# wdecoster/inquiSTR

Measured on AMD Instinct MI355X. Metric: loci/sec genotyped (inquiSTR call hot path, device-resident batch = L0), higher is better.
Workload: dtype u32/i64; 1 GPU; unphased100k: 100000 loci/GPU x 30 reads x ~200 CIGAR ops, --unphased, device-resident SoA (L0); loci_per_gpu=100000, pairs_per_gpu=3000000, cigar_ops_per_gpu=600007253, minlen=5, support=3, total_loci=100000

## Files before the change

inquistr_amd/csrc/capi.hip:

```cpp
#include <hip/hip_runtime.h>

#include <algorithm>
#include <cmath>
#include <cstdio>
#include <cstring>
#include <new>
#include <string>
#include <thread>
#include <vector>

#include "../../include/inquistr_hip.h"
#include "cigar_walk.h"
#include "ctx.h"
#include "evidence.h"
#include "front_kernels.h"
#include "kernels.h"
#include "locus_motifs.h"
#include "read_calls.h"
#include "read_motifs.h"
#include "read_seqs.h"

using namespace inq;

namespace inq {
// ... 66 lines not shown
    b.cap = got;
    return INQ_OK;
}

int upload(inq_ctx *c, hipStream_t s, std::initializer_list<Upload> ups) {
    for (const Upload &u : ups) {
        const int rc = ensure(c, *u.d, u.bytes);
        if (rc != INQ_OK) return rc;
        if (u.bytes) HIP_TRY(c, hipMemcpyAsync(u.d->p, u.h, u.bytes, hipMemcpyHostToDevice, s));
    }
    return INQ_OK;
}

int status_to_code(uint32_t st) {
    if (st & ST_HINT) return INQ_ERR_ARG;
    if (st & ST_LOCUS) return INQ_ERR_LOCUS;
    if (st & ST_INDEX) return INQ_ERR_INDEX;
    if (st & ST_CIGAR_OP) return INQ_ERR_CIGAR_OP;
    if (st & ST_RANGE) return INQ_ERR_RANGE;
    if (st & ST_PHASE) return INQ_ERR_PHASE;
    if (st & ST_AUX) return INQ_ERR_AUX;
    if (st & ST_INTERNAL) return INQ_ERR_HIP;
    return INQ_OK;
}

int status_readback(inq_ctx *c, DevStatus *dst, hipStream_t s) {
    HIP_TRY(c, hipMemcpyAsync(dst, c->d_status, sizeof(DevStatus), hipMemcpyDeviceToHost, s));
    HIP_TRY(c, hipMemsetAsync(&c->d_status->err, 0, sizeof(unsigned int), s));
    HIP_TRY(c, hipMemsetAsync(&c->d_status->ties, 0, sizeof(unsigned long long), s));
    return INQ_OK;
}

DevBatch device_batch(const void *cigar, const void *reads, const void *pair_read, const void *off, const void *lstart, const void *lend,
                      uint64_t n_reads, uint64_t n_cigar_words, uint64_t n_pairs, uint64_t n_loci, uint32_t minlen, uint32_t support,
                      uint32_t unphased, void *p1, void *p2, void *pair_call, void *pair_bits) {
    DevBatch d;
    d.b = {n_reads, n_cigar_words, n_pairs, n_loci, (const uint32_t *)cigar, (const inq_read_t *)reads, (const uint32_t *)pair_read,
           (const uint64_t *)off, (const uint32_t *)lstart, (const uint32_t *)lend, minlen, support, unphased, 0u};
    d.r = {(double *)p1, (double *)p2, (int64_t *)pair_call, (uint8_t *)pair_bits, 0};
    return d;
}

static int timing_begin(inq_ctx *c, hipStream_t s, EvTriple **ev) {
    *ev = nullptr;
    if (!c->timing) return INQ_OK;
    if (c->ev_used == c->ev_pool.size()) {
        EvTriple t;
        HIP_TRY(c, hipEventCreate(&t.e0));
        HIP_TRY(c, hipEventCreate(&t.e1));
        HIP_TRY(c, hipEventCreate(&t.e2));
        c->ev_pool.push_back(t);
    }
    *ev = &c->ev_pool[c->ev_used++];
    HIP_TRY(c, hipEventRecord((*ev)->e0, s));
    return INQ_OK;
}

}

extern "C" {

int inq_abi_version(void) { return INQ_ABI_VERSION; }

const char *inq_strerror(int code) {
    switch (code) {
    case INQ_OK: return "ok";
    case INQ_ERR_ARG: return "invalid argument (null pointer, inconsistent sizes or non-monotone offsets)";
    case INQ_ERR_SUPPORT_ZERO: return "support must be >= 1";
    case INQ_ERR_PHASE: return "a read passing the phased filter has HP outside {0,1,2}";
    case INQ_ERR_CIGAR_OP: return "CIGAR op code above 8";
    case INQ_ERR_LOCUS: return "locus start < 10 or end < start";
    case INQ_ERR_RANGE: return "read position plus reference span does not fit 31 bits";
    case INQ_ERR_INDEX: return "pair or CIGAR index outside the batch buffers";
    case INQ_ERR_HIP: return "HIP runtime error";
    case INQ_ERR_NOMEM: return "out of device memory";
    case INQ_ERR_INFLATE: return "a BGZF block does not inflate to its recorded size (corrupt or truncated BAM)";
    case INQ_ERR_BAM: return "corrupt BAM record chain, or records not coordinate-sorted";
    case INQ_ERR_AUX: return "HP aux of a fetched read is neither C nor i, or the SA aux of a kept read with a soft clip cannot be parsed (the reference panics)";
    case INQ_ERR_NO_DEVICE: return "no gfx950 (MI355X) device available; this library has no CPU fallback";
    default: return "unknown error";
    }
}

static void apply_default_options(inq_ctx *c);
static bool default_option(const char *key, int64_t *value);

int inq_ctx_create_early(int device_id, inq_ctx_t **out, volatile int *stage_ready) {
    if (!out) return INQ_ERR_ARG;
    *out = nullptr;
    if (stage_ready) *stage_ready = 0;
    int n = 0;
    HostClock clock("[inq ctx]");
    if (hipGetDeviceCount(&n) != hipSuccess || n <= 0) return INQ_ERR_NO_DEVICE;
    clock.lap("hipGetDeviceCount (runtime init)");
    if (device_id < 0 || device_id >= n) return INQ_ERR_ARG;
    hipDeviceProp_t prop;
    if (hipGetDeviceProperties(&prop, device_id) != hipSuccess) return INQ_ERR_HIP;
    if (std::strncmp(prop.gcnArchName, "gfx950", 6) != 0) return INQ_ERR_NO_DEVICE;
    inq_ctx *c = new (std::nothrow) inq_ctx();
    if (!c) return INQ_ERR_NOMEM;
    c->device = device_id;
    c->n_cus = (uint32_t)std::max(prop.multiProcessorCount, 1);
    c->grid_tail = std::min<uint32_t>(c->grid_tail, c->n_cus);
    c->backend = std::string("hip:") + prop.gcnArchName + ":" + prop.name;
    bool published = false;
    auto fail = [&](int code) {
// ... 124 lines not shown
    if (!x.kept_off != !x.kept || ((uintptr_t)x.kept & 15u) || ((uintptr_t)x.kept_off & 7u)) return INQ_ERR_ARG;
    if (x.kept && b->n_pairs && (!r->pair_call || !r->pair_bits)) return INQ_ERR_ARG;
    if (x.names.recs && (!x.kept || !x.names.off || !x.name_off || ((uintptr_t)x.names.recs & 7u))) return INQ_ERR_ARG;
    if (x.seqs.recs && (!x.kept || !x.kept_pair || !x.seqs.off || !x.seq_qbeg || !x.seq_len || ((uintptr_t)x.seqs.recs & 7u))) return INQ_ERR_ARG;
    if (((uintptr_t)b->cigar & 15u) || ((uintptr_t)b->reads & 15u)) return INQ_ERR_ARG;
    HIP_TRY(c, hipSetDevice(c->device));
    hipStream_t s = hip_stream ? (hipStream_t)hip_stream : c->stream;
    const uint64_t blocks = (b->n_loci + 3) / 4;
    const uint32_t per_xcd = (uint32_t)((blocks + 7) / 8);
    const uint32_t grid_small = per_xcd * 8u;
    const uint32_t shard_cap = (grid_small / kListShards + 1u) * 4u;
    if ((rc = ensure(c, c->worklist, (size_t)shard_cap * kListShards * kListKinds * 4)) != INQ_OK) return rc;
    if ((rc = ensure(c, c->sval, (size_t)b->n_pairs * 8)) != INQ_OK) return rc;
    if ((rc = ensure(c, c->smeta, (size_t)b->n_pairs)) != INQ_OK) return rc;
    const uint32_t hint = c->call_hint ? c->call_hint : c->max_reads_hint;
    const bool deep_possible = b->n_pairs > kGridSelectMin && !(hint && hint <= kGridSelectMin);
    if (deep_possible && (rc = ensure(c, c->deep, deep_select_scratch_bytes(b->n_pairs))) != INQ_OK) return rc;
    const uint64_t ev_list_cap = x.evidence && b->n_pairs > kEvidenceWaveMax && !(hint && hint <= kEvidenceWaveMax) ? evidence_list_cap(b->n_pairs) : 0;
    if (x.evidence && (rc = ensure(c, c->evwork, evidence_scratch_bytes(ev_list_cap))) != INQ_OK) return rc;
    if (x.kept && b->n_pairs && (rc = ensure(c, c->rctiles, read_call_scratch_bytes(b->n_pairs))) != INQ_OK) return rc;

    KArgs a;
    a.cigar4 = (const uint4 *)b->cigar;
    a.reads = (const uint4 *)b->reads;
    a.pair_read = b->pair_read;
    a.locus_pair_off = b->locus_pair_off;
    a.locus_start = b->locus_start;
    a.locus_end = b->locus_end;
    a.n_reads = b->n_reads;
    a.n_cigar4 = b->n_cigar_words / 4;
    a.n_pairs = b->n_pairs;
    a.n_loci = b->n_loci;
    a.minlen = b->minlen;
    a.support = b->support;
    a.phase1 = r->phase1;
    a.phase2 = r->phase2;
    a.pair_call = r->pair_call;
    a.pair_bits = r->pair_bits;
    a.status = c->d_status;
    a.worklist = (uint32_t *)c->worklist.p;
    a.sval = (int64_t *)c->sval.p;
    a.smeta = (uint8_t *)c->smeta.p;
    a.blocks_per_xcd = per_xcd;
    a.shard_cap = shard_cap;
    c->call_hint = 0;
    a.max_reads_hint = hint;
    a.locus_flags = x.flags;

    const bool nt = c->nt_loads < 0 ? (b->n_pairs <= b->n_reads) : (c->nt_loads != 0);
    EvTriple *ev;
    if ((rc = timing_begin(c, s, &ev)) != INQ_OK) return rc;
    if (x.flags) HIP_TRY(c, hipMemsetAsync(x.flags, 0, (size_t)b->n_loci, s));
    if (x.evidence) HIP_TRY(c, hipMemsetAsync(c->evwork.p, 0, sizeof(EvidenceWork), s));
    launch_locus_call(a, b->unphased != 0, nt, grid_small, c->grid_medium, c->grid_tail, s, ev ? ev->e1 : nullptr, deep_possible ? c->deep.p : nullptr);
    HIP_TRY(c, hipGetLastError());
    const PairView view{b->locus_pair_off, r->pair_bits, r->pair_call, b->pair_read, (const uint32_t *)b->reads, b->n_reads, b->n_pairs, b->n_loci};
    if (x.evidence) {
        EvidenceWork *const work = (EvidenceWork *)c->evwork.p;
        launch_evidence(EvidenceArgs{view, x.evidence, work, (EvidenceSlice *)(work + 1), ev_list_cap}, b->unphased != 0, c->n_cus * 4u, s);
        HIP_TRY(c, hipGetLastError());
    }
    if (x.kept && !b->n_pairs) HIP_TRY(c, hipMemsetAsync(x.kept_off, 0, (size_t)(b->n_loci + 1) * 8, s));
    if (x.kept && b->n_pairs) {
        uint64_t *const tile_base = (uint64_t *)c->rctiles.p;
        launch_read_calls(ReadCallArgs{view, x.kept_off, x.kept, (uint32_t *)(tile_base + read_call_tiles(b->n_pairs) + 1), tile_base, x.kept_pair},
                          b->unphased != 0, s);
        HIP_TRY(c, hipGetLastError());
    }
    const uint64_t *const n_kept = x.kept_off ? x.kept_off + b->n_loci : nullptr;
    auto place_runs = [&](const auto &runs, auto &&records) {
        if (!runs.recs) return hipSuccess;
        if (!b->n_pairs) return hipMemsetAsync(runs.off, 0, 8, s);
        records();
        launch_scan_run_bytes(runs.recs, n_kept, runs.off, b->n_pairs, runs.off + b->n_pairs + 1, s);
        return hipGetLastError();
    };
    const auto origins = [&] { launch_read_origins(ReadOriginArgs{x.kept, n_kept, view.read_words, b->n_reads, x.name_off, x.names.recs, b->n_pairs}, c->grid_side, s); };
    const auto slices = [&] { launch_read_seq_records(ReadSeqArgs{x.kept_pair, n_kept, x.seq_qbeg, x.seq_len, x.seqs.recs, b->n_pairs}, c->grid_side, s); };
    HIP_TRY(c, place_runs(x.names, origins));
    HIP_TRY(c, place_runs(x.seqs, slices));
    const KeptSlices kept{x.kept_pair, n_kept, x.kept_off, b->n_loci, x.seq_bytes, x.seq_n_bytes, x.seq_off, x.seq_len, b->n_pairs, b->n_pairs};
    if (x.locus_found && !b->n_pairs) HIP_TRY(c, hipMemsetAsync(x.locus_found, 0, (size_t)b->n_loci * sizeof(inq_locus_motif_t), s));
    if (x.locus_found && b->n_pairs) {
        launch_locus_motifs(LocusMotifArgs{kept, x.motif_given, x.locus_found, x.motif_use}, c->grid_side, s);
        HIP_TRY(c, hipGetLastError());
    }
    if (x.motifs && b->n_pairs) {
        launch_read_motifs(ReadMotifArgs{kept, x.motif_word, x.motifs}, c->grid_side, s);
        HIP_TRY(c, hipGetLastError());
    }
    if (ev) HIP_TRY(c, hipEventRecord(ev->e2, s));
    return INQ_OK;
}

int inq_call_batch_device(inq_ctx_t *c, const inq_batch_t *b, inq_result_t *r, void *hip_stream) {
    return inq_call_batch_device_flags(c, b, r, nullptr, hip_stream);
}

int inq_call_batch_device_flags(inq_ctx_t *c, const inq_batch_t *b, inq_result_t *r, uint8_t *d_locus_flags, void *hip_stream) {
    return inq_call_batch_device_evidence(c, b, r, d_locus_flags, nullptr, hip_stream);
}

int inq_call_batch_device_evidence(inq_ctx_t *c, const inq_batch_t *b, inq_result_t *r, uint8_t *d_locus_flags, inq_locus_evidence_t *d_evidence,
                                   void *hip_stream) {
    return inq_call_batch_device_reads(c, b, r, d_locus_flags, d_evidence, nullptr, nullptr, hip_stream);
}

int inq_call_batch_device_reads(inq_ctx_t *c, const inq_batch_t *b, inq_result_t *r, uint8_t *d_locus_flags, inq_locus_evidence_t *d_evidence,
                                uint64_t *d_kept_off, inq_read_call_t *d_kept, void *hip_stream) {
    return guarded([&] { return enqueue_batch(c, b, r, hip_stream, LocusExtras{d_locus_flags, d_evidence, d_kept_off, d_kept}); });
}

int inq_ctx_status(inq_ctx_t *c, uint64_t *n_tie_loci) {
    if (!c) return INQ_ERR_ARG;
    HIP_TRY(c, hipSetDevice(c->device));
    HIP_TRY(c, hipDeviceSynchronize());
    const int rc = status_readback(c, c->h_status, c->stream);
    if (rc != INQ_OK) return rc;
    HIP_TRY(c, hipStreamSynchronize(c->stream));
    if (n_tie_loci) *n_tie_loci = c->h_status->ties;
    return status_to_code(c->h_status->err);
}

static int call_batch_impl(inq_ctx_t *c, const inq_batch_t *b, inq_result_t *r, const HostExtras &h) {
    if (!c) return INQ_ERR_ARG;
    extras_reset(c);
    int rc = check_scalars(b, r);
    if (rc != INQ_OK) return rc;
    uint64_t max_reads = 0;
    if (b->n_loci) {
        const uint64_t *const off = b->locus_pair_off;
        if (off[0] != 0 || off[b->n_loci] != b->n_pairs || !offsets_ok(off, b->n_loci, b->n_pairs)) return INQ_ERR_ARG;
        for (uint64_t j = 0; j < b->n_loci; ++j) {
            if (!locus_ok(b->locus_start[j], b->locus_end[j])) return INQ_ERR_LOCUS;
            max_reads = std::max<uint64_t>(max_reads, b->locus_pair_off[j + 1] - b->locus_pair_off[j]);
        }
    }
    r->n_tie_loci = 0;
    if (b->n_loci == 0) {
        extras_finish(c, 0, 0, h, 0);
        return INQ_OK;
    }
    HIP_TRY(c, hipSetDevice(c->device));
    hipStream_t s = c->stream;
// ... 158 lines not shown
        if (firth_when) {
            launch_assoc_firth(a, s);
            HIP_TRY(c, hipGetLastError());
        }
        if (ev) {
            HIP_TRY(c, hipEventRecord(ev->e1, s));
            HIP_TRY(c, hipEventRecord(ev->e2, s));
        }
        HIP_TRY(c, hipMemcpyAsync(rows + r0, c->arows.p, a.n_rows * sizeof(inq_assoc_row_t), hipMemcpyDeviceToHost, s));
        if (firth_when) HIP_TRY(c, hipMemcpyAsync(firth + r0, c->afirth.p, a.n_rows * sizeof(inq_assoc_firth_row_t), hipMemcpyDeviceToHost, s));
    }
    HIP_TRY(c, hipStreamSynchronize(s));
    return INQ_OK;
}

int inq_assoc_rows(inq_ctx_t *c, const float *values, uint64_t n_rows, uint32_t n_samples, const double *y, const double *cov, uint32_t k,
                   int outcome, int str_mode, double missing_cutoff, inq_assoc_row_t *rows) {
    return guarded([&] { return assoc_rows_impl(c, values, n_rows, n_samples, y, cov, k, outcome, str_mode, missing_cutoff, rows); });
}

int inq_assoc_rows_firth(inq_ctx_t *c, const float *values, uint64_t n_rows, uint32_t n_samples, const double *y, const double *cov,
                         uint32_t k, int str_mode, double missing_cutoff, int when, inq_assoc_row_t *rows, inq_assoc_firth_row_t *firth) {
    if (when != INQ_ASSOC_FIRTH_FALLBACK && when != INQ_ASSOC_FIRTH_ALWAYS) return INQ_ERR_ARG;
    return guarded([&] { return assoc_rows_impl(c, values, n_rows, n_samples, y, cov, k, INQ_ASSOC_BINARY, str_mode, missing_cutoff, rows, when, firth); });
}

int inq_ctx_timing_enable(inq_ctx_t *c, int on) {
    if (!c) return INQ_ERR_ARG;
    c->timing = on != 0;
    return INQ_OK;
}

int inq_ctx_timing_reset(inq_ctx_t *c) {
    if (!c) return INQ_ERR_ARG;
    HIP_TRY(c, hipSetDevice(c->device));
    HIP_TRY(c, hipDeviceSynchronize());
    c->ev_used = 0;
    return INQ_OK;
}

int inq_ctx_timing_read(inq_ctx_t *c, int which, double *total_ms, uint64_t *launches) {
    if (!c || which < 0 || which > 2) return INQ_ERR_ARG;
    HIP_TRY(c, hipSetDevice(c->device));
    if (which == 2) {
        HIP_TRY(c, hipDeviceSynchronize());
        const double ms = span_last_inflate_ms(c->span);
        if (total_ms) *total_ms = ms < 0 ? 0.0 : ms;
        if (launches) *launches = ms < 0 ? 0u : 1u;
        return INQ_OK;
    }
    double tot = 0.0;
    for (size_t i = 0; i < c->ev_used; ++i) {
        EvTriple &e = c->ev_pool[i];
        HIP_TRY(c, hipEventSynchronize(e.e2));
        float ms = 0.f;
        HIP_TRY(c, hipEventElapsedTime(&ms, e.e0, which == 0 ? e.e2 : e.e1));
        tot += (double)ms;
    }
    if (total_ms) *total_ms = tot;
    if (launches) *launches = (uint64_t)c->ev_used;
    return INQ_OK;
}

static std::mutex g_defaults_mu;
static std::vector<std::pair<std::string, int64_t>> g_defaults;

int inq_default_option(const char *key, int64_t value) {
    if (!key) return INQ_ERR_ARG;
    try {
        inq_ctx probe;
        probe.n_cus = 256;
        const int rc = inq_ctx_set_option(&probe, key, value);
        if (rc != INQ_OK) return rc;
        std::lock_guard<std::mutex> g(g_defaults_mu);
        for (auto &kv : g_defaults)
            if (kv.first == key) {
                kv.second = value;
                return INQ_OK;
            }
        g_defaults.emplace_back(key, value);
        return INQ_OK;
    } catch (...) {
        return INQ_ERR_NOMEM;
    }
}

static bool default_option(const char *key, int64_t *value) {
    std::lock_guard<std::mutex> g(g_defaults_mu);
    for (auto &kv : g_defaults)
        if (kv.first == key) {
            if (value) *value = kv.second;
            return true;
        }
    return false;
}
int inq_default_option_get(const char *key, int64_t *value) {
    if (!key) return INQ_ERR_ARG;
    try {
        return default_option(key, value) ? INQ_OK : INQ_ERR_ARG;
    } catch (...) {
        return INQ_ERR_NOMEM;
    }
}

static void apply_default_options(inq_ctx *c) {
    std::vector<std::pair<std::string, int64_t>> d;
    {
        std::lock_guard<std::mutex> g(g_defaults_mu);
        d = g_defaults;
// ... 123 lines not shown
```

inquistr_amd/csrc/cigar_walk.h:

```cpp
#pragma once
#include <type_traits>

#include "wave_primitives.h"

namespace inq {

typedef unsigned int u32x4 __attribute__((ext_vector_type(4)));

constexpr uint32_t ST_INDEX = 1u, ST_CIGAR_OP = 2u, ST_RANGE = 4u, ST_PHASE = 8u, ST_LOCUS = 16u, ST_HINT = 32u, ST_AUX = 64u,
                   ST_INTERNAL = 128u;

constexpr uint32_t PM_CLIP = 1u, PM_FETCHED = 2u, PM_KEPT = 4u;
constexpr int PM_GRP_SHIFT = 4;
constexpr uint32_t PM_CHOSEN = 64u;

constexpr uint32_t RB_UNMAPPED = 1u, RB_REVERSE = 2u, RB_HAS_HP = 4u, RB_IS_2D = 8u, RB_SA_PANIC = 16u;

constexpr int kQueueCap = 128;

struct Window {
    uint32_t se;
    uint32_t ee;
    uint32_t se1;
    uint32_t width;
// ... 53 lines not shown
    if (lane < cnt) {
        uint32_t ri = b.pair_read[first + (uint64_t)lane];
        if ((uint64_t)ri < b.n_reads) {
            uint4 r = b.reads[ri];
            uint64_t n4 = ((uint64_t)r.y + 3u) >> 2;
            if (r.y < 0x10000000u && (uint64_t)r.x + n4 <= b.n_cigar4) {
                m.off4 = r.x;
                m.nc = r.y | ((r.w & (RB_IS_2D << 8)) ? 0x80000000u : 0u);
                m.pos = r.z;
                m.misc = r.w;
                valid = true;
            } else {
                status |= ST_INDEX;
            }
        } else {
            status |= ST_INDEX;
        }
    }
    return m;
}

__device__ __forceinline__ uint32_t meta_stage_a(const BatchView &b, uint64_t first, int cnt, int lane) {
    return lane < cnt ? b.pair_read[first + (uint64_t)lane] : 0xffffffffu;
}
__device__ __forceinline__ uint4 meta_stage_b(const BatchView &b, uint32_t ri) {
    return (uint64_t)ri < b.n_reads ? b.reads[ri] : make_uint4(0u, 0xffffffffu, 0u, 0u);
}
__device__ __forceinline__ PairMeta meta_stage_c(const BatchView &b, const uint4 r, int cnt, int lane, uint32_t &status,
                                                  bool &valid) {
    PairMeta m{0u, 0u, 0u, 0u};
    valid = false;
    if (lane < cnt) {
        const uint64_t n4 = ((uint64_t)r.y + 3u) >> 2;
        if (r.y < 0x10000000u && (uint64_t)r.x + n4 <= b.n_cigar4) {
            m.off4 = r.x;
            m.nc = r.y | ((r.w & (RB_IS_2D << 8)) ? 0x80000000u : 0u);
            m.pos = r.z;
            m.misc = r.w;
            valid = true;
        } else {
            status |= ST_INDEX;
        }
    }
    return m;
}

constexpr uint32_t kConsume = 0x18Du;

__device__ __forceinline__ uint32_t ref_advance(uint32_t op, uint32_t len) {
    return len & (uint32_t)__builtin_amdgcn_sbfe((int)kConsume, op, 1u);
}
constexpr uint32_t kConsume32 = kConsume | (kConsume << 16);
__device__ __forceinline__ uint32_t ref_advance_raw(uint32_t w) {
    return (w >> 4) & (uint32_t)__builtin_amdgcn_sbfe((int)kConsume32, w, 1u);
}
constexpr uint32_t kBadOp32 = 0xFE00FE00u;
__device__ __forceinline__ uint32_t bad_ops(const u32x4 w) {
    return (kBadOp32 >> (w.x & 31u)) | (kBadOp32 >> (w.y & 31u)) | (kBadOp32 >> (w.z & 31u)) | (kBadOp32 >> (w.w & 31u));
}
__device__ __forceinline__ void advance4(const u32x4 w, uint32_t &e1, uint32_t &e2, uint32_t &e3, uint32_t &tot) {
    e1 = ref_advance_raw(w.x), e2 = e1 + ref_advance_raw(w.y);
    e3 = e2 + ref_advance_raw(w.z), tot = e3 + ref_advance_raw(w.w);
}

__device__ __forceinline__ void drain_queue(WaveLds &L, uint32_t &qcount, const Window &W, int lane) {
    __builtin_amdgcn_wave_barrier();
    for (uint32_t base = 0; base < qcount; base += 64u) {
        const uint32_t e = base + (uint32_t)lane;
        if (e < qcount) {
            const u32x4 w = L.q[e].w;
            const uint2 info = L.q[e].info;
            const uint32_t rel = info.x;
            const uint32_t slot = info.y & 63u;
            const uint32_t cand_mask = (info.y & 64u) ? 0x06u : 0x16u;
            const uint32_t op0 = w.x & 15u, op1 = w.y & 15u, op2 = w.z & 15u, op3 = w.w & 15u;
            const uint32_t l0 = w.x >> 4, l1 = w.y >> 4, l2 = w.z >> 4, l3 = w.w >> 4;
            const uint32_t e1 = ref_advance(op0, l0), e2 = e1 + ref_advance(op1, l1), e3 = e2 + ref_advance(op2, l2);
            int32_t s = 0;
            uint32_t clip = 0;
#define INQ_OP(op, len, ee_)                                                                              \
    {                                                                                                     \
        const bool hit = ((cand_mask >> (op)) & 1u) && (len) > W.minlen && (rel + (ee_)) < W.width;        \
        const int32_t v = ((op) == 2u) ? -(int32_t)(len) : (int32_t)(len);                                \
        s += hit ? v : 0;                                                                                 \
        clip |= (hit && (op) == 4u) ? 1u : 0u;                                                            \
    }
            INQ_OP(op0, l0, 0u)
            INQ_OP(op1, l1, e1)
            INQ_OP(op2, l2, e2)
            INQ_OP(op3, l3, e3)
#undef INQ_OP
            if (s != 0) atomicAdd(&L.acc[slot], (unsigned long long)(long long)s);
            if (clip) atomicOr(&L.flags[slot], 1u);
        }
    }
    qcount = 0;
    __builtin_amdgcn_wave_barrier();
}

__device__ __forceinline__ bool push_window_lanes(WaveLds &L, uint32_t &qcount, bool inw, const u32x4 w, uint32_t x,
                                                  uint32_t tot, uint32_t info, uint32_t info_mask) {
    const uint64_t mask = ballot64(inw);
    if (mask) {
        QueueEntry *const tail = &L.q[qcount];
        if (inw) {
            const uint32_t idx = __builtin_amdgcn_mbcnt_hi((uint32_t)(mask >> 32), __builtin_amdgcn_mbcnt_lo((uint32_t)mask, 0u));
            tail[idx].w = w;
// ... 367 lines not shown
```

inquistr_amd/csrc/ctx.h:

```cpp
#pragma once
#include <hip/hip_runtime.h>

#include <array>
#include <chrono>
#include <cstdio>
#include <cstdlib>
#include <initializer_list>
#include <mutex>
#include <new>
#include <string>
#include <utility>
#include <vector>

#include "../../include/inquistr_hip.h"
#include "kernels.h"

namespace inq {

struct DevBuf {
    void *p = nullptr;
    size_t cap = 0;
};

struct EvTriple {
    hipEvent_t e0, e1, e2;
};

struct KeptRuns {
    DevBuf recs, off, bytes;
    uint64_t n_recs = 0, n_bytes = 0;
    auto bufs() { return std::array{&recs, &off, &bytes}; }
};

struct SpanState;

}

struct inq_ctx {
    int device = -1;
    hipStream_t stream = nullptr;
    std::string backend, last_err;
    inq::DevStatus *d_status = nullptr;
    inq::DevStatus *h_status = nullptr;
    inq::DevBuf worklist, sval, smeta, deep;
    inq::DevBuf cigar, reads, pair_read, off, lstart, lend, p1, p2, pcall, pbits, lflags;
    inq::DevBuf levidence, evwork;
    inq::DevBuf rctiles, rcoff, rckept;
    uint64_t read_calls_total = 0;
    inq::KeptRuns rnames, rseqs;
    inq::DevBuf rkeptpair;
    inq::DevBuf rmotifs, rmotifword;
    uint64_t read_motifs_total = 0;
    inq::DevBuf rlocusmotif, rmotifuse;
    inq::DevBuf ovalues, olen, oflags, okeep, otrans;
    inq::DevBuf avalues, ay, acov, atcoef, arows;
    inq::DevBuf aminmu, afirth;
    auto bufs() {
        std::vector<inq::DevBuf *> all{&worklist, &sval, &smeta, &deep, &cigar, &reads, &pair_read, &off, &lstart, &lend, &p1, &p2, &pcall, &pbits,
                                       &lflags, &levidence, &evwork, &rctiles, &rcoff, &rckept, &rkeptpair, &rmotifs, &rmotifword, &rlocusmotif, &rmotifuse, &ovalues, &olen, &oflags, &okeep, &otrans,
                                       &avalues, &ay, &acov, &atcoef, &arows, &aminmu, &afirth};
        for (inq::KeptRuns *k : {&rnames, &rseqs})
            for (inq::DevBuf *b : k->bufs()) all.push_back(b);
        return all;
    }
    uint32_t n_cus = 0;
    uint32_t grid_tail = 256;
    uint32_t grid_medium = 4096;
    uint32_t grid_side = 0;
    uint32_t max_reads_hint = 0;
    uint32_t call_hint = 0;
    int nt_loads = -1;
    bool timing = false;
    bool verify_crc = true;
    int inflate_tokens = 0;
    int inflate_lit_pairs = -1;
    int inflate_ahead = 1;
    int outlier_tile = 1;
    uint64_t assoc_tile_rows = 0;
// ... 144 lines not shown
```

inquistr_amd/csrc/kernels.h:

```cpp
#pragma once
#include <hip/hip_runtime.h>
#include <stdint.h>

#include "../../include/inquistr_hip.h"

namespace inq {

constexpr int kListShards = 32;
constexpr int kListKinds = 3;
constexpr uint32_t kWalkSplit = 16384;
constexpr uint32_t kReduceInPlace = 2048;

struct DevStatus {
    unsigned int err;
    unsigned int pad;
    struct alignas(128) Counter {
        unsigned int n;
    } list_count[kListKinds][kListShards];
    unsigned long long ties;
    struct alignas(128) Word {
        unsigned int v;
    } bar_count, bar_abort, exit_ticket;
};

struct KArgs {
    const uint4 *cigar4;
    const uint4 *reads;
    const uint32_t *pair_read;
    const uint64_t *locus_pair_off;
    const uint32_t *locus_start;
    const uint32_t *locus_end;
    uint64_t n_reads, n_cigar4, n_pairs, n_loci;
    uint32_t minlen, support;
    double *phase1, *phase2;
    int64_t *pair_call;
    uint8_t *pair_bits;
    DevStatus *status;
    uint32_t *worklist;
    int64_t *sval;
    uint8_t *smeta;
    uint32_t blocks_per_xcd;
    uint32_t shard_cap;
    uint32_t max_reads_hint;
    uint8_t *locus_flags;
};

void launch_locus_call(const KArgs &a, bool unphased, bool nt_loads, uint32_t grid_small, uint32_t grid_medium,
                       uint32_t grid_tail, hipStream_t s, hipEvent_t ev_mid, void *deep_scratch);

constexpr uint32_t kGridSelectMin = 65536;
size_t deep_select_scratch_bytes(uint64_t n_pairs);
void launch_locus_tail(const KArgs &k, bool unphased, void *scratch, uint64_t n_pairs, uint32_t grid, hipStream_t s);

}
```

inquistr_amd/csrc/kernels.hip:

```cpp
#include <hip/hip_runtime.h>
#include <stdint.h>

#include "cigar_walk.h"
#include "deep_reduce.h"
#include "kernels.h"

namespace inq {

__device__ __forceinline__ bool before(int64_t vj, int j, int64_t v, int i) {
    return vj < v || (vj == v && j < i);
}

__device__ __forceinline__ uint32_t xcd_remap(uint32_t b, uint32_t per_xcd) { return (b & 7u) * per_xcd + (b >> 3); }

template <int E>
struct Masks {
    uint64_t m[E];
    __device__ __forceinline__ uint32_t count() const {
        uint32_t c = 0;
#pragma unroll
        for (int s = 0; s < E; ++s) c += (uint32_t)__popcll(m[s]);
        return c;
    }
    __device__ __forceinline__ bool any() const {
// ... 20 lines not shown
            key_desc[s] = (int32_t)(((uint32_t)(int32_t)v[s] << IDX_BITS) | ((uint32_t)(E * 64 - 1) - idx));
        }
    }
    __device__ __forceinline__ void rank_asc(const Masks<E> &mask, uint32_t (&r)[E]) const {
#pragma unroll
        for (int t = 0; t < E; ++t) r[t] = 0;
#pragma unroll
        for (int s = 0; s < E; ++s) {
            for (uint64_t mk = mask.m[s]; mk; mk &= mk - 1) {
                const int j = __builtin_ctzll(mk);
                if (FIT) {
                    const int32_t kj = (int32_t)readlane_u32((uint32_t)key_asc[s], j);
#pragma unroll
                    for (int t = 0; t < E; ++t) r[t] += (kj < key_asc[t]) ? 1u : 0u;
                } else {
                    const int64_t vj = readlane_i64(val[s], j);
#pragma unroll
                    for (int t = 0; t < E; ++t) r[t] += before(vj, s * 64 + j, val[t], t * 64 + lane) ? 1u : 0u;
                }
            }
        }
    }
    __device__ __forceinline__ void rank_desc(const Masks<E> &mask, uint32_t (&r)[E]) const {
#pragma unroll
        for (int t = 0; t < E; ++t) r[t] = 0;
#pragma unroll
        for (int s = 0; s < E; ++s) {
            for (uint64_t mk = mask.m[s]; mk; mk &= mk - 1) {
                const int j = __builtin_ctzll(mk);
                if (FIT) {
                    const int32_t kj = (int32_t)readlane_u32((uint32_t)key_desc[s], j);
#pragma unroll
                    for (int t = 0; t < E; ++t) r[t] += (kj > key_desc[t]) ? 1u : 0u;
                } else {
                    const int64_t vj = readlane_i64(val[s], j);
#pragma unroll
                    for (int t = 0; t < E; ++t)
                        r[t] += (vj > val[t] || (vj == val[t] && s * 64 + j < t * 64 + lane)) ? 1u : 0u;
                }
            }
        }
    }
    __device__ __forceinline__ int64_t pick(const Masks<E> &mask, const uint32_t (&r)[E], uint32_t want) const {
        int64_t out = 0;
#pragma unroll
        for (int s = 0; s < E; ++s) {
            const uint64_t b = ballot64(((mask.m[s] >> lane) & 1ull) && r[s] == want);
            if (b) out = readlane_i64(val[s], __builtin_ctzll(b));
        }
        return out;
    }
};

template <bool FIT, int E>
__device__ __forceinline__ double median_in_lanes(const Masks<E> &g, const Masks<E> &clip, const LaneOrder<FIT, E> &o,
                                                  uint32_t support) {
    const int lane = o.lane;
    const uint32_t ng = g.count();
    if (!group_live(ng, support)) return qnan();
    Masks<E> cm, chosen;
#pragma unroll
    for (int s = 0; s < E; ++s) {
        cm.m[s] = g.m[s] & clip.m[s];
        chosen.m[s] = g.m[s] & ~clip.m[s];
    }
    const GroupPlan P = plan_group(ng, chosen.count(), support);
    if (P.take > 0u) {
        uint32_t drank[E];
        o.rank_desc(cm, drank);
#pragma unroll
        for (int s = 0; s < E; ++s) chosen.m[s] |= ballot64(((cm.m[s] >> lane) & 1ull) && drank[s] < P.take);
    }
    uint32_t arank[E];
    o.rank_asc(chosen, arank);
    const int64_t vhi = o.pick(chosen, arank, P.M / 2u);
    const int64_t vlo = (P.M & 1u) ? vhi : o.pick(chosen, arank, P.M / 2u - 1u);
    return median_finish(vlo, vhi, P.M);
}

template <bool UNPHASED, bool FIT, int E>
__device__ __forceinline__ void reduce_locus_in_lanes(const int64_t (&val)[E], const uint32_t (&meta)[E], int lane,
                                                      uint32_t support, double &out1, double &out2, bool &tie) {
    const LaneOrder<FIT, E> o(val, lane);
    Masks<E> kept, clip;
#pragma unroll
    for (int s = 0; s < E; ++s) {
        kept.m[s] = ballot64(meta[s] & PM_KEPT);
        clip.m[s] = ballot64((meta[s] & PM_KEPT) && (meta[s] & PM_CLIP));
    }
    tie = false;
    if (UNPHASED) {
        const uint32_t mcount = kept.count();
        const uint32_t ks = mcount / 2u;
        uint32_t rank[E];
        o.rank_asc(kept, rank);
        if (!clip.any()) {
            auto med = [&](uint32_t base, uint32_t cnt) -> double {
                if (!group_live(cnt, support)) return qnan();
                const int64_t vhi = o.pick(kept, rank, base + cnt / 2u);
                const int64_t vlo = (cnt & 1u) ? vhi : o.pick(kept, rank, base + cnt / 2u - 1u);
                return median_finish(vlo, vhi, cnt);
            };
            out1 = med(0u, ks);
            out2 = med(ks, mcount - ks);
        } else {
            Masks<E> g1, g2;
#pragma unroll
            for (int s = 0; s < E; ++s) {
                g1.m[s] = ballot64(((kept.m[s] >> lane) & 1ull) && rank[s] < ks);
                g2.m[s] = kept.m[s] & ~g1.m[s];
            }
            if (ks >= 1u && ks < mcount) {
                const int64_t va = o.pick(kept, rank, ks - 1u), vb = o.pick(kept, rank, ks);
                if (va == vb) {
                    bool has_clip = false, has_span = false;
#pragma unroll
                    for (int s = 0; s < E; ++s) {
                        const uint64_t eq = ballot64(((kept.m[s] >> lane) & 1ull) && val[s] == va);
                        has_clip |= (eq & clip.m[s]) != 0ull;
                        has_span |= (eq & ~clip.m[s]) != 0ull;
                    }
                    tie = has_clip && has_span;
                }
            }
            out1 = median_in_lanes<FIT, E>(g1, clip, o, support);
            out2 = median_in_lanes<FIT, E>(g2, clip, o, support);
        }
    } else {
        Masks<E> g1, g2;
#pragma unroll
        for (int s = 0; s < E; ++s) {
            g1.m[s] = ballot64(((meta[s] >> PM_GRP_SHIFT) & 3u) == 1u);
            g2.m[s] = ballot64(((meta[s] >> PM_GRP_SHIFT) & 3u) == 2u);
        }
        out1 = median_in_lanes<FIT, E>(g1, clip, o, support);
        out2 = median_in_lanes<FIT, E>(g2, clip, o, support);
    }
}

template <bool UNPHASED, int AUX, int E>
__device__ __forceinline__ void wave_locus(const KArgs &a, uint64_t j, uint64_t p0, int n, uint32_t start, uint32_t end,
                                           int lane, WaveLds &L) {
    const Window W = make_window(start, end, a.minlen);
    BatchView b{a.cigar4, a.reads, a.pair_read, a.n_reads, a.n_cigar4};
    uint32_t status = 0;
    int64_t val[E];
// ... 118 lines not shown
    SortLds<(int)kReduceInPlace> sort;
};

template <bool UNPHASED, int AUX>
__device__ __forceinline__ void walk_part(const KArgs &a, MidLds &lds, const uint32_t (&cnt)[kListShards], const uint32_t (&cnt2)[kListShards], int lane,
                                          uint32_t wave) {
    BatchView b{a.cigar4, a.reads, a.pair_read, a.n_reads, a.n_cigar4};
    uint32_t total = 0;
    for (int k = 0; k < kListShards; ++k) total += cnt[k];
    for (uint32_t item = blockIdx.x; item < total; item += gridDim.x) {
        const uint64_t j = worklist_locus(a, cnt, 1u, item);
        const uint64_t p0 = a.locus_pair_off[j];
        const uint32_t n = (uint32_t)(a.locus_pair_off[j + 1] - p0);
        walk_locus<UNPHASED, AUX>(a, b, j, p0, n, 1u, 0u, lane, wave, lds.wave[wave]);
        if (n <= kReduceInPlace) {
            asm volatile("s_waitcnt vmcnt(0)" ::: "memory");
            __syncthreads();
            sort_reduce_locus<UNPHASED, (int)kReduceInPlace, true>(a, j, p0, n, lds.sort, nullptr);
        }
        __syncthreads();
    }
    total = 0;
    for (int k = 0; k < kListShards; ++k) total += cnt2[k];
    if (total == 0u) return;
    const uint32_t per_item = max(1u, gridDim.x / total), groups = gridDim.x / per_item;
    const uint32_t my_group = blockIdx.x / per_item, my_rank = blockIdx.x % per_item;
    if (my_group >= groups) return;
    for (uint32_t item = my_group; item < total; item += groups) {
        const uint64_t j = worklist_locus(a, cnt2, 2u, item);
        const uint64_t p0 = a.locus_pair_off[j];
        const uint64_t n64 = a.locus_pair_off[j + 1] - p0;
        if (n64 > 0xffffffffull) continue;
        walk_locus<UNPHASED, AUX>(a, b, j, p0, (uint32_t)n64, per_item, my_rank, lane, wave, lds.wave[wave]);
    }
}

template <bool UNPHASED, int AUX>
__global__ __launch_bounds__(256) __attribute__((amdgpu_waves_per_eu(5))) void locus_call_mid_walk(KArgs a) {
    __shared__ MidLds lds;
    __shared__ uint32_t cnt[kListKinds][kListShards];
    const int lane = threadIdx.x & 63;
    const uint32_t wave = __builtin_amdgcn_readfirstlane(threadIdx.x >> 6);
    if (threadIdx.x < kListKinds * kListShards) cnt[threadIdx.x / kListShards][threadIdx.x % kListShards] = a.status->list_count[threadIdx.x / kListShards][threadIdx.x % kListShards].n;
    __syncthreads();
    medium_part<UNPHASED, AUX>(a, lds.wave, cnt[0], lane, wave);
    walk_part<UNPHASED, AUX>(a, lds, cnt[1], cnt[2], lane, wave);
}

__global__ void clear_lists(KArgs a) {
    if (threadIdx.x < kListKinds * kListShards) a.status->list_count[threadIdx.x / kListShards][threadIdx.x % kListShards].n = 0u;
}

template <bool UNPHASED, int AUX>
static void launch_t(const KArgs &a, uint32_t grid_small, uint32_t grid_medium, uint32_t grid_tail, hipStream_t s,
                     hipEvent_t ev_mid, void *deep_scratch) {
    if (grid_small) hipLaunchKernelGGL((locus_call_small<UNPHASED, AUX>), dim3(grid_small), dim3(256), 0, s, a);
    if (ev_mid) (void)hipEventRecord(ev_mid, s);
    const uint32_t h = a.max_reads_hint;
    if (h && h <= 64u) return;
    hipLaunchKernelGGL((locus_call_mid_walk<UNPHASED, AUX>), dim3(grid_medium), dim3(256), 0, s, a);
    if (h && h <= 64u * kMediumSlots) {
        hipLaunchKernelGGL(clear_lists, dim3(1), dim3(128), 0, s, a);
        return;
    }
    launch_locus_tail(a, UNPHASED, deep_scratch, a.n_pairs, grid_tail, s);
}

void launch_locus_call(const KArgs &a, bool unphased, bool nt_loads, uint32_t grid_small, uint32_t grid_medium,
                       uint32_t grid_tail, hipStream_t s, hipEvent_t ev_mid, void *deep_scratch) {
    if (unphased) {
        if (nt_loads)
            launch_t<true, 2>(a, grid_small, grid_medium, grid_tail, s, ev_mid, deep_scratch);
        else
            launch_t<true, 0>(a, grid_small, grid_medium, grid_tail, s, ev_mid, deep_scratch);
    } else {
        if (nt_loads)
            launch_t<false, 2>(a, grid_small, grid_medium, grid_tail, s, ev_mid, deep_scratch);
        else
            launch_t<false, 0>(a, grid_small, grid_medium, grid_tail, s, ev_mid, deep_scratch);
    }
}

__global__ void preload_locus_kernel() {}
void preload_locus(hipStream_t s) { hipLaunchKernelGGL(preload_locus_kernel, dim3(1), dim3(64), 0, s); }

}
```

inquistr_amd/csrc/wave_primitives.h:

```cpp
#pragma once
#include <hip/hip_runtime.h>
#include <stdint.h>

namespace inq {

constexpr int kWave = 64;
constexpr int kRowLanes = 16;

constexpr int DPP_ROW_SHR1 = 0x111;
constexpr int DPP_ROW_SHR2 = 0x112;
constexpr int DPP_ROW_SHR4 = 0x114;
constexpr int DPP_ROW_SHR8 = 0x118;
constexpr int DPP_ROW_BCAST15 = 0x142;
constexpr int DPP_ROW_BCAST31 = 0x143;

__device__ __forceinline__ int lane_id() { return (int)__builtin_amdgcn_mbcnt_hi(~0u, __builtin_amdgcn_mbcnt_lo(~0u, 0u)); }

template <int CTRL>
__device__ __forceinline__ uint32_t dpp_shr_zero(uint32_t x) {
    return (uint32_t)__builtin_amdgcn_update_dpp(0, (int)x, CTRL, 0xf, 0xf, true);
}
template <int CTRL>
__device__ __forceinline__ uint64_t dpp_shr_zero_u64(uint64_t x) {
    return (uint64_t)dpp_shr_zero<CTRL>((uint32_t)x) | (uint64_t)dpp_shr_zero<CTRL>((uint32_t)(x >> 32)) << 32;
}
template <int CTRL, int ROW_MASK>
__device__ __forceinline__ uint32_t dpp_bcast(uint32_t x) {
    return (uint32_t)__builtin_amdgcn_update_dpp(0, (int)x, CTRL, ROW_MASK, 0xf, false);
}

__device__ __forceinline__ uint32_t row_inclusive_scan_u32(uint32_t x) {
    x += dpp_shr_zero<DPP_ROW_SHR1>(x);
    x += dpp_shr_zero<DPP_ROW_SHR2>(x);
    x += dpp_shr_zero<DPP_ROW_SHR4>(x);
    x += dpp_shr_zero<DPP_ROW_SHR8>(x);
    return x;
}
__device__ __forceinline__ uint64_t row_inclusive_scan_u64(uint64_t x) {
    x += dpp_shr_zero_u64<DPP_ROW_SHR1>(x);
    x += dpp_shr_zero_u64<DPP_ROW_SHR2>(x);
    x += dpp_shr_zero_u64<DPP_ROW_SHR4>(x);
    x += dpp_shr_zero_u64<DPP_ROW_SHR8>(x);
    return x;
}
__device__ __forceinline__ uint32_t row_last(uint32_t x) { return (uint32_t)__builtin_amdgcn_ds_swizzle((int)x, 0x10 | (0x0f << 5)); }
__device__ __forceinline__ uint64_t row_last_u64(uint64_t x) { return (uint64_t)row_last((uint32_t)x) | (uint64_t)row_last((uint32_t)(x >> 32)) << 32; }
__device__ __forceinline__ uint32_t row_or(uint32_t x) {
    x |= dpp_shr_zero<DPP_ROW_SHR1>(x);
    x |= dpp_shr_zero<DPP_ROW_SHR2>(x);
    x |= dpp_shr_zero<DPP_ROW_SHR4>(x);
    x |= dpp_shr_zero<DPP_ROW_SHR8>(x);
    return x;
}
__device__ __forceinline__ uint64_t row_max_u64(uint64_t x) {
    const auto larger = [](uint64_t o, uint64_t v) { return o > v ? o : v; };
    x = larger(dpp_shr_zero_u64<DPP_ROW_SHR1>(x), x);
    x = larger(dpp_shr_zero_u64<DPP_ROW_SHR2>(x), x);
    x = larger(dpp_shr_zero_u64<DPP_ROW_SHR4>(x), x);
    x = larger(dpp_shr_zero_u64<DPP_ROW_SHR8>(x), x);
    return x;
}

__device__ __forceinline__ uint32_t wave_inclusive_scan_u32(uint32_t x) {
    x = row_inclusive_scan_u32(x);
    x += dpp_bcast<DPP_ROW_BCAST15, 0xa>(x);
    x += dpp_bcast<DPP_ROW_BCAST31, 0xc>(x);
    return x;
}

__device__ __forceinline__ uint32_t readlane_u32(uint32_t v, int l) {
    return (uint32_t)__builtin_amdgcn_readlane((int)v, l);
}
__device__ __forceinline__ int64_t readlane_i64(int64_t v, int l) {
    uint32_t lo = readlane_u32((uint32_t)v, l);
    uint32_t hi = readlane_u32((uint32_t)((uint64_t)v >> 32), l);
    return (int64_t)(((uint64_t)hi << 32) | lo);
}
extern "C" __device__ int inq_llvm_writelane_i32(int value, int lane, int old) __asm("llvm.amdgcn.writelane.i32");
__device__ __forceinline__ uint32_t writelane_u32(uint32_t old, uint32_t value, int l) {
    return (uint32_t)inq_llvm_writelane_i32((int)value, l, (int)old);
}
__device__ __forceinline__ uint64_t ballot64(bool p) { return __builtin_amdgcn_ballot_w64(p); }

__device__ __forceinline__ uint32_t wave_sum_u32(uint32_t x) { return readlane_u32(wave_inclusive_scan_u32(x), kWave - 1); }
__device__ __forceinline__ uint64_t wave_sum_u64(uint64_t x) {
    for (int d = 1; d < kWave; d *= 2) x += __shfl_xor((unsigned long long)x, d, kWave);
    return x;
}

constexpr uint32_t kGridCap = 1u << 16;
inline uint32_t capped_grid(uint64_t tiles, uint32_t cap = kGridCap) { return (uint32_t)(tiles < cap ? tiles : cap); }
inline uint32_t side_grid(uint64_t tiles, uint32_t grid_side, uint32_t cap = kGridCap) {
    return capped_grid(tiles, grid_side && grid_side < cap ? grid_side : cap);
}

}
```

Baseline: 510.1 million loci/s.

## Use wave bitonic sort for unphased median and skip redundant end event

```diff
diff --git a/inquistr_amd/csrc/capi.hip b/inquistr_amd/csrc/capi.hip
--- a/inquistr_amd/csrc/capi.hip
+++ b/inquistr_amd/csrc/capi.hip
@@ -142,6 +142,7 @@
         c->ev_pool.push_back(t);
     }
     *ev = &c->ev_pool[c->ev_used++];
+    (*ev)->one_kernel = false;
     HIP_TRY(c, hipEventRecord((*ev)->e0, s));
     return INQ_OK;
 }
@@ -372,7 +373,7 @@
     if ((rc = timing_begin(c, s, &ev)) != INQ_OK) return rc;
     if (x.flags) HIP_TRY(c, hipMemsetAsync(x.flags, 0, (size_t)b->n_loci, s));
     if (x.evidence) HIP_TRY(c, hipMemsetAsync(c->evwork.p, 0, sizeof(EvidenceWork), s));
-    launch_locus_call(a, b->unphased != 0, nt, grid_small, c->grid_medium, c->grid_tail, s, ev ? ev->e1 : nullptr, deep_possible ? c->deep.p : nullptr);
+    const bool more_kernels = launch_locus_call(a, b->unphased != 0, nt, grid_small, c->grid_medium, c->grid_tail, s, ev ? ev->e1 : nullptr, deep_possible ? c->deep.p : nullptr);
     HIP_TRY(c, hipGetLastError());
     const PairView view{b->locus_pair_off, r->pair_bits, r->pair_call, b->pair_read, (const uint32_t *)b->reads, b->n_reads, b->n_pairs, b->n_loci};
     if (x.evidence) {
@@ -409,7 +410,11 @@
         launch_read_motifs(ReadMotifArgs{kept, x.motif_word, x.motifs}, c->grid_side, s);
         HIP_TRY(c, hipGetLastError());
     }
-    if (ev) HIP_TRY(c, hipEventRecord(ev->e2, s));
+    const bool side_outputs = x.evidence || x.kept || x.names.recs || x.seqs.recs || x.locus_found || x.motifs;
+    if (ev) {
+        ev->one_kernel = !more_kernels && !side_outputs;
+        if (!ev->one_kernel) HIP_TRY(c, hipEventRecord(ev->e2, s));
+    }
     return INQ_OK;
 }
 
@@ -674,9 +679,10 @@
     double tot = 0.0;
     for (size_t i = 0; i < c->ev_used; ++i) {
         EvTriple &e = c->ev_pool[i];
-        HIP_TRY(c, hipEventSynchronize(e.e2));
+        const hipEvent_t last = e.one_kernel ? e.e1 : e.e2;
+        HIP_TRY(c, hipEventSynchronize(last));
         float ms = 0.f;
-        HIP_TRY(c, hipEventElapsedTime(&ms, e.e0, which == 0 ? e.e2 : e.e1));
+        HIP_TRY(c, hipEventElapsedTime(&ms, e.e0, which == 0 ? last : e.e1));
         tot += (double)ms;
     }
     if (total_ms) *total_ms = tot;
diff --git a/inquistr_amd/csrc/cigar_walk.h b/inquistr_amd/csrc/cigar_walk.h
--- a/inquistr_amd/csrc/cigar_walk.h
+++ b/inquistr_amd/csrc/cigar_walk.h
@@ -129,7 +129,7 @@
 }
 constexpr uint32_t kConsume32 = kConsume | (kConsume << 16);
 __device__ __forceinline__ uint32_t ref_advance_raw(uint32_t w) {
-    return (w >> 4) & (uint32_t)__builtin_amdgcn_sbfe((int)kConsume32, w, 1u);
+    return __builtin_amdgcn_ubfe(w, 4u, (uint32_t)__builtin_amdgcn_sbfe((int)kConsume32, w, 1u));
 }
 constexpr uint32_t kBadOp32 = 0xFE00FE00u;
 __device__ __forceinline__ uint32_t bad_ops(const u32x4 w) {
diff --git a/inquistr_amd/csrc/ctx.h b/inquistr_amd/csrc/ctx.h
--- a/inquistr_amd/csrc/ctx.h
+++ b/inquistr_amd/csrc/ctx.h
@@ -24,6 +24,7 @@
 
 struct EvTriple {
     hipEvent_t e0, e1, e2;
+    bool one_kernel = false;
 };
 
 struct KeptRuns {
diff --git a/inquistr_amd/csrc/kernels.h b/inquistr_amd/csrc/kernels.h
--- a/inquistr_amd/csrc/kernels.h
+++ b/inquistr_amd/csrc/kernels.h
@@ -45,7 +45,7 @@
     uint8_t *locus_flags;
 };
 
-void launch_locus_call(const KArgs &a, bool unphased, bool nt_loads, uint32_t grid_small, uint32_t grid_medium,
+bool launch_locus_call(const KArgs &a, bool unphased, bool nt_loads, uint32_t grid_small, uint32_t grid_medium,
                        uint32_t grid_tail, hipStream_t s, hipEvent_t ev_mid, void *deep_scratch);
 
 constexpr uint32_t kGridSelectMin = 65536;
diff --git a/inquistr_amd/csrc/kernels.hip b/inquistr_amd/csrc/kernels.hip
--- a/inquistr_amd/csrc/kernels.hip
+++ b/inquistr_amd/csrc/kernels.hip
@@ -96,6 +96,71 @@
     }
 };
 
+constexpr uint64_t keep_max_mask(int kk, int j) {
+    uint64_t m = 0;
+    for (int l = 0; l < kWave; ++l)
+        if (((l & kk) == 0) != ((l & j) == 0)) m |= 1ull << l;
+    return m;
+}
+template <int KK, int J>
+__device__ __forceinline__ int32_t bitonic_stage(int32_t k, int lane) {
+    const int32_t p = (int32_t)lane_xor<J>((uint32_t)k, lane);
+    return __builtin_amdgcn_inverse_ballot_w64(ballot64(p < k) ^ keep_max_mask(KK, J)) ? p : k;
+}
+template <int KK, int J, int KK_LAST>
+__device__ __forceinline__ int32_t bitonic_stages(int32_t k, int lane) {
+    k = bitonic_stage<KK, J>(k, lane);
+    if constexpr (J > 1)
+        return bitonic_stages<KK, J / 2, KK_LAST>(k, lane);
+    else if constexpr (KK < KK_LAST)
+        return bitonic_stages<KK * 2, KK, KK_LAST>(k, lane);
+    else
+        return k;
+}
+__device__ __forceinline__ int32_t wave_sort_asc(int32_t k, int lane, bool upper_all_max) {
+    k = bitonic_stages<2, 1, 32>(k, lane);
+    if (!upper_all_max) k = bitonic_stages<64, 32, 64>(k, lane);
+    return k;
+}
+
+struct SortSim {
+    int32_t k[kWave];
+};
+constexpr SortSim sort_sim_run(SortSim a, int kk_last) {
+    for (int kk = 2; kk <= kk_last; kk *= 2)
+        for (int j = kk / 2; j >= 1; j /= 2) {
+            const uint64_t keep_max = keep_max_mask(kk, j);
+            SortSim r = a;
+            for (int l = 0; l < kWave; ++l) {
+                const int32_t p = a.k[l ^ j];
+                if ((p < a.k[l]) != (((keep_max >> l) & 1ull) != 0ull)) r.k[l] = p;
+            }
+            a = r;
+        }
+    return a;
+}
+constexpr bool sort_sim_ok(int pattern, uint64_t pads) {
+    SortSim a{};
+    for (int l = 0; l < kWave; ++l) {
+        const int32_t v = pattern == 0 ? l - 20 : pattern == 1 ? 43 - l : pattern == 2 ? ((l & 1) ? -5 : 7) : 3;
+        a.k[l] = ((pads >> l) & 1ull) ? INT32_MAX : (int32_t)(((uint32_t)v << 6) | (uint32_t)l);
+    }
+    const SortSim s = sort_sim_run(a, (pads >> 32) == 0xffffffffull ? 32 : 64);
+    for (int l = 0; l + 1 < kWave; ++l)
+        if (s.k[l] > s.k[l + 1]) return false;
+    for (int l = 0; l < kWave; ++l) {
+        int in = 0, out = 0;
+        for (int t = 0; t < kWave; ++t) in += a.k[t] == a.k[l], out += s.k[t] == a.k[l];
+        if (in != out) return false;
+    }
+    return true;
+}
+constexpr bool sort_sim_all(uint64_t pads) { return sort_sim_ok(0, pads) && sort_sim_ok(1, pads) && sort_sim_ok(2, pads) && sort_sim_ok(3, pads); }
+static_assert(sort_sim_all(0ull), "21 stages, every lane kept");
+static_assert(sort_sim_all(0xaaaaaaaaaaaaaaaaull) && sort_sim_all(0x00000000ffffffffull) && sort_sim_all(0x8000000000000001ull), "21 stages, pads");
+static_assert(sort_sim_all(0xffffffff00000000ull) && sort_sim_all(0xffffffffc0000003ull) && sort_sim_all(0xffffffff55555555ull), "15 stages");
+static_assert(sort_sim_all(~0ull) && sort_sim_all(~1ull) && sort_sim_all(~(1ull << 63)), "nothing or one read kept");
+
 template <bool FIT, int E>
 __device__ __forceinline__ double median_in_lanes(const Masks<E> &g, const Masks<E> &clip, const LaneOrder<FIT, E> &o,
                                                   uint32_t support) {
@@ -136,6 +201,21 @@
     if (UNPHASED) {
         const uint32_t mcount = kept.count();
         const uint32_t ks = mcount / 2u;
+        if constexpr (FIT && E == 1) {
+            if (!clip.any()) {
+                const int32_t sorted = wave_sort_asc(((kept.m[0] >> lane) & 1ull) ? o.key_asc[0] : INT32_MAX, lane, (kept.m[0] >> 32) == 0ull);
+                auto med = [&](uint32_t base, uint32_t cnt) -> double {
+                    if (!group_live(cnt, support)) return qnan();
+                    const auto at = [&](uint32_t r) { return (int64_t)((int32_t)readlane_u32((uint32_t)sorted, (int)r) >> LaneOrder<FIT, E>::IDX_BITS); };
+                    const int64_t vhi = at(base + cnt / 2u);
+                    const int64_t vlo = (cnt & 1u) ? vhi : at(base + cnt / 2u - 1u);
+                    return median_finish(vlo, vhi, cnt);
+                };
+                out1 = med(0u, ks);
+                out2 = med(ks, mcount - ks);
+                return;
+            }
+        }
         uint32_t rank[E];
         o.rank_asc(kept, rank);
         if (!clip.any()) {
@@ -360,33 +440,28 @@
 }
 
 template <bool UNPHASED, int AUX>
-static void launch_t(const KArgs &a, uint32_t grid_small, uint32_t grid_medium, uint32_t grid_tail, hipStream_t s,
+static bool launch_t(const KArgs &a, uint32_t grid_small, uint32_t grid_medium, uint32_t grid_tail, hipStream_t s,
                      hipEvent_t ev_mid, void *deep_scratch) {
     if (grid_small) hipLaunchKernelGGL((locus_call_small<UNPHASED, AUX>), dim3(grid_small), dim3(256), 0, s, a);
     if (ev_mid) (void)hipEventRecord(ev_mid, s);
     const uint32_t h = a.max_reads_hint;
-    if (h && h <= 64u) return;
+    if (h && h <= 64u) return false;
     hipLaunchKernelGGL((locus_call_mid_walk<UNPHASED, AUX>), dim3(grid_medium), dim3(256), 0, s, a);
     if (h && h <= 64u * kMediumSlots) {
         hipLaunchKernelGGL(clear_lists, dim3(1), dim3(128), 0, s, a);
-        return;
+        return true;
     }
     launch_locus_tail(a, UNPHASED, deep_scratch, a.n_pairs, grid_tail, s);
-}
-
-void launch_locus_call(const KArgs &a, bool unphased, bool nt_loads, uint32_t grid_small, uint32_t grid_medium,
+    return true;
+}
+
+bool launch_locus_call(const KArgs &a, bool unphased, bool nt_loads, uint32_t grid_small, uint32_t grid_medium,
                        uint32_t grid_tail, hipStream_t s, hipEvent_t ev_mid, void *deep_scratch) {
-    if (unphased) {
-        if (nt_loads)
-            launch_t<true, 2>(a, grid_small, grid_medium, grid_tail, s, ev_mid, deep_scratch);
-        else
-            launch_t<true, 0>(a, grid_small, grid_medium, grid_tail, s, ev_mid, deep_scratch);
-    } else {
-        if (nt_loads)
-            launch_t<false, 2>(a, grid_small, grid_medium, grid_tail, s, ev_mid, deep_scratch);
-        else
-            launch_t<false, 0>(a, grid_small, grid_medium, grid_tail, s, ev_mid, deep_scratch);
-    }
+    if (unphased)
+        return nt_loads ? launch_t<true, 2>(a, grid_small, grid_medium, grid_tail, s, ev_mid, deep_scratch)
+                        : launch_t<true, 0>(a, grid_small, grid_medium, grid_tail, s, ev_mid, deep_scratch);
+    return nt_loads ? launch_t<false, 2>(a, grid_small, grid_medium, grid_tail, s, ev_mid, deep_scratch)
+                    : launch_t<false, 0>(a, grid_small, grid_medium, grid_tail, s, ev_mid, deep_scratch);
 }
 
 __global__ void preload_locus_kernel() {}
diff --git a/inquistr_amd/csrc/wave_primitives.h b/inquistr_amd/csrc/wave_primitives.h
--- a/inquistr_amd/csrc/wave_primitives.h
+++ b/inquistr_amd/csrc/wave_primitives.h
@@ -45,6 +45,14 @@
 }
 __device__ __forceinline__ uint32_t row_last(uint32_t x) { return (uint32_t)__builtin_amdgcn_ds_swizzle((int)x, 0x10 | (0x0f << 5)); }
 __device__ __forceinline__ uint64_t row_last_u64(uint64_t x) { return (uint64_t)row_last((uint32_t)x) | (uint64_t)row_last((uint32_t)(x >> 32)) << 32; }
+template <int J>
+__device__ __forceinline__ uint32_t lane_xor(uint32_t x, int lane) {
+    static_assert(J == 1 || J == 2 || J == 4 || J == 8 || J == 16 || J == 32, "one lane bit");
+    if constexpr (J < 32)
+        return (uint32_t)__builtin_amdgcn_ds_swizzle((int)x, 0x1f | (J << 10));
+    else
+        return (uint32_t)__builtin_amdgcn_ds_bpermute((lane ^ 32) << 2, (int)x);
+}
 __device__ __forceinline__ uint32_t row_or(uint32_t x) {
     x |= dpp_shr_zero<DPP_ROW_SHR1>(x);
     x |= dpp_shr_zero<DPP_ROW_SHR2>(x);
```

Measured after the change: 534.3 million loci/s, median of 6. 4.7% higher.
